# google/lyra

Hardware: NVIDIA H100
Metric: 20ms-frame encode+decode throughput (frames/s) @16kHz (higher is better)
Workload: dtype f32+i8 (decoder fp32 GEMMs: split tf32 on tensor cores)

## Files before the change

include/lyra_b200.h:

```cpp
#ifndef LYRA_B200_H_
#define LYRA_B200_H_

#include <stdint.h>

#ifdef __cplusplus
extern "C" {
#endif

#define LYRA_B200_OK 0
#define LYRA_B200_EINVAL (-1)
#define LYRA_B200_ENODEV (-2)
#define LYRA_B200_EMODEL (-3)

#define LYRA_B200_HOP 320
#define LYRA_B200_NUM_FEATURES 64
#define LYRA_B200_MAX_BITS 184
#define LYRA_B200_MAX_STAGES 46

typedef struct lyra_b200_ctx lyra_b200_ctx;

int lyra_b200_create(const char* model_dir, int device, int max_streams, lyra_b200_ctx** out);
#define LYRA_B200_ROLE_ENCODER 1
#define LYRA_B200_ROLE_DECODER 2
int lyra_b200_create_ex(const char* model_dir, int device, int max_streams, int roles, lyra_b200_ctx** out);
// ... 78 lines not shown
                              int32_t* d_indices );
int lyra_b200_dequantize_device(lyra_b200_ctx* ctx, int n, const uint8_t* d_packets, int num_bits, float* d_features);
int lyra_b200_generate_device(lyra_b200_ctx* ctx, int n, const float* d_features , int16_t* d_pcm );
int lyra_b200_logmel_device(lyra_b200_ctx* ctx, int bank, int n, const int16_t* d_pcm, int num_mel_bins, float* d_out);
int lyra_b200_noise_estimate_device(lyra_b200_ctx* ctx, int n, float* d_noise_estimate ,
                                    uint8_t* d_is_noise );
int lyra_b200_cng_generate_device(lyra_b200_ctx* ctx, int n, const float* d_features , int16_t* d_pcm );
int lyra_b200_resample_device(lyra_b200_ctx* ctx, int to_internal, int n, int external_rate_hz, const int16_t* d_in, int in_samples,
                              int16_t* d_out, int out_stride, int32_t* d_out_counts );
int lyra_b200_set_active_mask(lyra_b200_ctx* ctx, const uint8_t* d_active);
#define LYRA_B200_STATS_WORDS 8
#define LYRA_B200_STAT_HOPS 0
#define LYRA_B200_STAT_SAT_OUT 1
#define LYRA_B200_STAT_ENERGY 2
#define LYRA_B200_STAT_LEVEL 3
#define LYRA_B200_STAT_EMPTY 4
#define LYRA_B200_STAT_BITS 5
#define LYRA_B200_STAT_RECEIVED 4
#define LYRA_B200_STAT_CN_HOPS 5
#define LYRA_B200_STAT_EVENTS 6
int lyra_b200_set_stats(lyra_b200_ctx* ctx, int enable);
int lyra_b200_read_stats(lyra_b200_ctx* ctx, int role, const int32_t* stream_ids, int n, uint64_t* stats , int clear);
int lyra_b200_read_stats_device(lyra_b200_ctx* ctx, int role, int n, uint64_t* d_stats , int clear);
int lyra_b200_synchronize(lyra_b200_ctx* ctx);
int lyra_b200_set_split(lyra_b200_ctx* ctx, int parts);
#define LYRA_B200_DECODER_EXACT 0
#define LYRA_B200_DECODER_TENSOR 1
int lyra_b200_set_decoder_mode(lyra_b200_ctx* ctx, int mode);
int lyra_b200_decoder_mode(const lyra_b200_ctx* ctx);
int lyra_b200_set_blocking_sync(lyra_b200_ctx* ctx, int enable);
int lyra_b200_set_priority(lyra_b200_ctx* ctx, int priority);
int lyra_b200_set_graphs(lyra_b200_ctx* ctx, int enable);
uint64_t lyra_b200_graph_replays(const lyra_b200_ctx* ctx);
uint64_t lyra_b200_launch_count(const lyra_b200_ctx* ctx);

#define LYRA_B200_NUM_KERNELS 8
int lyra_b200_profile_enable(lyra_b200_ctx* ctx, int enable);
int lyra_b200_profile_read(lyra_b200_ctx* ctx, double* ms_sum, uint64_t* launches);

#ifdef __cplusplus
}
#endif
#endif
```

lyra_b200/_capi.py:

```python
import ctypes as C
import os

import numpy as np

_HERE = os.path.dirname(os.path.abspath(__file__))
PRODUCT_SO = os.path.join(_HERE, "liblyra_b200.so")
MODEL_DIR = os.path.join(_HERE, "model_coeffs")

OK, EINVAL, ENODEV, EMODEL = 0, -1, -2, -3
HOP = 320
STATS_WORDS = 8
STAT_HOPS, STAT_SAT_OUT, STAT_ENERGY, STAT_LEVEL = 0, 1, 2, 3
STAT_EMPTY, STAT_BITS = 4, 5
STAT_RECEIVED, STAT_CN_HOPS, STAT_EVENTS = 4, 5, 6
NUM_FEATURES = 64
MAX_STAGES = 46


class LyraB200Error(RuntimeError):
    def __init__(self, code, msg):
        super().__init__("lyra_b200 error %d: %s" % (code, msg))
        self.code = code


class CApi:
    def __init__(self, so_path):
        if not os.path.exists(so_path):
            raise FileNotFoundError(
                "%s not found: the CUDA extension is not built (python -c 'import __graft_entry__ as g; g.build()')" % so_path)
        L = C.CDLL(so_path)
        vp, ci = C.c_void_p, C.c_int
        sig = {
            "lyra_b200_create": (ci, [C.c_char_p, ci, ci, C.POINTER(vp)]),
            "lyra_b200_create_ex": (ci, [C.c_char_p, ci, ci, ci, C.POINTER(vp)]),
            "lyra_b200_destroy": (None, [vp]),
            "lyra_b200_last_error": (C.c_char_p, [vp]),
            "lyra_b200_max_streams": (ci, [vp]),
            "lyra_b200_tile_streams": (ci, [vp]),
            "lyra_b200_reset": (ci, [vp, vp, ci]),
            "lyra_b200_encode": (ci, [vp, vp, ci, vp, ci, vp]),
            "lyra_b200_decode": (ci, [vp, vp, ci, vp, vp, ci, vp]),
            "lyra_b200_extract_features": (ci, [vp, vp, ci, vp, vp]),
            "lyra_b200_quantize": (ci, [vp, ci, vp, ci, vp, vp]),
            "lyra_b200_dequantize": (ci, [vp, ci, vp, ci, vp]),
            "lyra_b200_generate": (ci, [vp, vp, ci, vp, vp]),
            "lyra_b200_logmel": (ci, [vp, ci, vp, ci, vp, ci, vp]),
            "lyra_b200_set_stream": (ci, [vp, vp]),
            "lyra_b200_encode_device": (ci, [vp, ci, vp, ci, vp]),
            "lyra_b200_decode_device": (ci, [vp, ci, vp, vp, ci, vp]),
            "lyra_b200_synchronize": (ci, [vp]),
            "lyra_b200_noise_update": (ci, [vp, vp, ci, vp, vp, vp, vp]),
            "lyra_b200_decode_track_noise": (ci, [vp, vp, ci, vp, vp, ci, vp, vp]),
            "lyra_b200_decode_track_noise_device": (ci, [vp, ci, vp, vp, ci, vp, vp]),
            "lyra_b200_noise_update_device": (ci, [vp, ci, vp, vp, vp, vp]),
            "lyra_b200_set_split": (ci, [vp, ci]),
            "lyra_b200_set_blocking_sync": (ci, [vp, ci]),
            "lyra_b200_set_graphs": (ci, [vp, ci]),
            "lyra_b200_set_priority": (ci, [vp, ci]),
            "lyra_b200_graph_replays": (C.c_uint64, [vp]),
            "lyra_b200_set_decoder_mode": (ci, [vp, ci]),
            "lyra_b200_decoder_mode": (ci, [vp]),
            "lyra_b200_launch_count": (C.c_uint64, [vp]),
            "lyra_b200_profile_enable": (ci, [vp, ci]),
            "lyra_b200_profile_read": (ci, [vp, vp, vp]),
            "lyra_b200_noise_estimate": (ci, [vp, vp, ci, vp, vp]),
            "lyra_b200_decode_plc": (ci, [vp, vp, ci, vp, vp, ci, vp, vp]),
            "lyra_b200_decode_plc_device": (ci, [vp, ci, vp, vp, ci, vp, vp]),
            "lyra_b200_plc_get_state": (ci, [vp, vp, ci, vp]),
            "lyra_b200_plc_set_state": (ci, [vp, vp, ci, vp]),
            "lyra_b200_cng_generate": (ci, [vp, vp, ci, vp, vp]),
            "lyra_b200_set_cng_seed": (ci, [vp, C.c_uint64]),
            "lyra_b200_encode_dtx": (ci, [vp, vp, ci, vp, ci, vp, vp]),
            "lyra_b200_encode_dtx_device": (ci, [vp, ci, vp, ci, vp, vp]),
            "lyra_b200_set_active_mask": (ci, [vp, vp]),
            "lyra_b200_set_stats": (ci, [vp, ci]),
            "lyra_b200_read_stats": (ci, [vp, ci, vp, ci, vp, ci]),
            "lyra_b200_read_stats_device": (ci, [vp, ci, ci, vp, ci]),
            "lyra_b200_resample": (ci, [vp, ci, vp, ci, ci, vp, ci, vp, ci, vp]),
            "lyra_b200_set_sample_rate": (ci, [vp, ci]),
            "lyra_b200_sample_rate": (ci, [vp]),
            "lyra_b200_set_stream_sample_rates": (ci, [vp, vp, ci, vp]),
            "lyra_b200_stream_sample_rates": (ci, [vp, vp, ci, vp]),
            "lyra_b200_set_stream_bits": (ci, [vp, ci, vp, ci, vp]),
            "lyra_b200_stream_bits": (ci, [vp, ci, vp, ci, vp]),
            "lyra_b200_set_stream_dtx": (ci, [vp, vp, ci, vp]),
            "lyra_b200_stream_dtx": (ci, [vp, vp, ci, vp]),
            "lyra_b200_stream_state_bytes": (ci, [vp]),
            "lyra_b200_export_streams": (ci, [vp, vp, ci, vp]),
            "lyra_b200_import_streams": (ci, [vp, vp, ci, vp]),
            "lyra_b200_copy_streams": (ci, [vp, vp, vp, ci]),
            "lyra_b200_align_streams": (ci, [vp, vp, vp, ci]),
            "lyra_b200_extract_features_device": (ci, [vp, ci, vp, vp]),
            "lyra_b200_quantize_device": (ci, [vp, ci, vp, ci, vp, vp]),
            "lyra_b200_dequantize_device": (ci, [vp, ci, vp, ci, vp]),
            "lyra_b200_generate_device": (ci, [vp, ci, vp, vp]),
            "lyra_b200_logmel_device": (ci, [vp, ci, ci, vp, ci, vp]),
            "lyra_b200_noise_estimate_device": (ci, [vp, ci, vp, vp]),
            "lyra_b200_cng_generate_device": (ci, [vp, ci, vp, vp]),
            "lyra_b200_resample_device": (ci, [vp, ci, ci, ci, vp, ci, vp, ci, vp]),
        }
        for name, (res, args) in sig.items():
            fn = getattr(L, name)
            fn.restype = res
            fn.argtypes = args
        self.lib = L
        self.path = so_path

    EXPORTS = ["lyra_b200_create", "lyra_b200_create_ex", "lyra_b200_destroy", "lyra_b200_last_error", "lyra_b200_max_streams",
               "lyra_b200_tile_streams", "lyra_b200_reset", "lyra_b200_encode", "lyra_b200_decode",
               "lyra_b200_extract_features", "lyra_b200_quantize", "lyra_b200_dequantize", "lyra_b200_generate",
               "lyra_b200_logmel", "lyra_b200_set_stream", "lyra_b200_encode_device", "lyra_b200_decode_device",
               "lyra_b200_synchronize", "lyra_b200_noise_update", "lyra_b200_noise_update_device", "lyra_b200_decode_track_noise",
               "lyra_b200_decode_track_noise_device", "lyra_b200_set_split", "lyra_b200_set_blocking_sync", "lyra_b200_set_graphs", "lyra_b200_set_priority", "lyra_b200_graph_replays", "lyra_b200_set_decoder_mode", "lyra_b200_decoder_mode", "lyra_b200_launch_count", "lyra_b200_profile_enable",
               "lyra_b200_profile_read", "lyra_b200_noise_estimate", "lyra_b200_decode_plc", "lyra_b200_decode_plc_device",
               "lyra_b200_plc_get_state", "lyra_b200_plc_set_state", "lyra_b200_cng_generate", "lyra_b200_set_cng_seed",
               "lyra_b200_encode_dtx", "lyra_b200_encode_dtx_device", "lyra_b200_set_active_mask", "lyra_b200_set_stats",
               "lyra_b200_read_stats", "lyra_b200_read_stats_device", "lyra_b200_resample", "lyra_b200_set_sample_rate",
               "lyra_b200_sample_rate", "lyra_b200_set_stream_sample_rates", "lyra_b200_stream_sample_rates", "lyra_b200_set_stream_bits",
               "lyra_b200_stream_bits", "lyra_b200_set_stream_dtx", "lyra_b200_stream_dtx", "lyra_b200_stream_state_bytes", "lyra_b200_export_streams", "lyra_b200_import_streams",
               "lyra_b200_copy_streams", "lyra_b200_align_streams", "lyra_b200_extract_features_device", "lyra_b200_quantize_device",
               "lyra_b200_dequantize_device", "lyra_b200_generate_device", "lyra_b200_logmel_device", "lyra_b200_noise_estimate_device",
               "lyra_b200_cng_generate_device", "lyra_b200_resample_device"]


_product = None


def load():
    global _product
    if _product is None:
        _product = CApi(PRODUCT_SO)
    return _product


def _ptr(a):
    return None if a is None else a.ctypes.data_as(C.c_void_p)


def _ids(stream_ids, n):
    if stream_ids is None:
        return None
    a = np.ascontiguousarray(stream_ids, dtype=np.int32)
    if a.size != n:
        raise ValueError("stream_ids must have one id per row")
    return a

# ... 318 lines not shown
                                                           C.c_void_p(d_indices or 0)))

    def dequantize_device(self, n, d_packets, num_bits, d_features):
        self._check(self.api.lib.lyra_b200_dequantize_device(self.h, n, C.c_void_p(d_packets), num_bits, C.c_void_p(d_features)))

    def generate_device(self, n, d_features, d_pcm):
        self._check(self.api.lib.lyra_b200_generate_device(self.h, n, C.c_void_p(d_features), C.c_void_p(d_pcm)))

    def logmel_device(self, n, d_pcm, d_out, num_mel_bins=160, bank=0):
        self._check(self.api.lib.lyra_b200_logmel_device(self.h, bank, n, C.c_void_p(d_pcm), num_mel_bins, C.c_void_p(d_out)))

    def noise_estimate_device(self, n, d_estimate, d_is_noise):
        self._check(self.api.lib.lyra_b200_noise_estimate_device(self.h, n, C.c_void_p(d_estimate or 0), C.c_void_p(d_is_noise or 0)))

    def cng_generate_device(self, n, d_features, d_pcm):
        self._check(self.api.lib.lyra_b200_cng_generate_device(self.h, n, C.c_void_p(d_features), C.c_void_p(d_pcm)))

    def resample_device(self, n, external_rate_hz, to_internal, d_in, in_samples, d_out, out_stride, d_counts=0):
        self._check(self.api.lib.lyra_b200_resample_device(self.h, 1 if to_internal else 0, n, int(external_rate_hz), C.c_void_p(d_in),
                                                           in_samples, C.c_void_p(d_out), out_stride, C.c_void_p(d_counts or 0)))

    def synchronize(self):
        self._check(self.api.lib.lyra_b200_synchronize(self.h))

    def set_decoder_mode(self, mode):
        self._check(self.api.lib.lyra_b200_set_decoder_mode(self.h, {"exact": 0, "tensor": 1}[mode]))

    def set_blocking_sync(self, enable):
        self._check(self.api.lib.lyra_b200_set_blocking_sync(self.h, 1 if enable else 0))

    def set_graphs(self, enable):
        self._check(self.api.lib.lyra_b200_set_graphs(self.h, 1 if enable else 0))

    def set_priority(self, priority):
        self._check(self.api.lib.lyra_b200_set_priority(self.h, int(priority)))

    def graph_replays(self):
        return int(self.api.lib.lyra_b200_graph_replays(self.h))

    def set_split(self, parts):
        self._check(self.api.lib.lyra_b200_set_split(self.h, int(parts)))

    KERNEL_NAMES = ["EncoderKernelA", "EncoderKernelB", "RvqEncodeKernel", "RvqDecodeKernel", "DecoderKernelC",
                    "DecoderKernelD", "LogMelKernel", "NoiseEstimatorKernel"]

    def profile_enable(self, enable=True):
        self._check(self.api.lib.lyra_b200_profile_enable(self.h, 1 if enable else 0))

    def profile_read(self):
        ms = (C.c_double * len(self.KERNEL_NAMES))()
        cnt = (C.c_uint64 * len(self.KERNEL_NAMES))()
        self._check(self.api.lib.lyra_b200_profile_read(self.h, ms, cnt))
        return {k: (ms[i], int(cnt[i])) for i, k in enumerate(self.KERNEL_NAMES)}
```

lyra_b200/csrc/aux_kernels.cuh:

```cuda
#pragma once

#include "kernel_prims.cuh"
#include "net_kernels.cuh"

namespace lyra_b200 {

constexpr int kRvqBitsPerStage = 4;

struct RowIo {
  const int* ids;
  int slot0, slots;
  const uint8_t* active;
  __device__ __forceinline__ int Stream(int slot) const { return ids ? ids[slot] : slot; }
  __device__ __forceinline__ bool SatOut(int slot) const { return active != nullptr && !active[slot]; }
};

struct StreamWords {
  const int* rate;
  int ctx_rate;
  const int* bits;
  const int* dtx_off;
  __device__ __forceinline__ int Rate(int stream) const {
    if (!rate) return ctx_rate;
    const int w = rate[stream];
    return w ? w : ctx_rate;
  }
  __device__ __forceinline__ int Stages(int stream, int nq) const {
    if (!bits) return nq;
    const int w = bits[stream];
    return w ? w / kRvqBitsPerStage : nq;
  }
  __device__ __forceinline__ bool DtxOff(int stream) const { return dtx_off != nullptr && dtx_off[stream] != 0; }
};

constexpr int kRvqThreads = 128;
constexpr int kRvqSlotsPerBlock = kRvqThreads / 16;

__global__ void __launch_bounds__(kRvqThreads)
RvqEncodeKernel(const uint8_t* __restrict__ blob, RvqParams P, const __grid_constant__ RowIo io, const __grid_constant__ StreamWords words,
                const float* __restrict__ features, int nq, uint8_t* __restrict__ packets, int packet_bytes, int* __restrict__ indices_out,
                const uint8_t* __restrict__ skip) {
  unsigned char* smem = LYRA_DYN_SMEM();
  float* cbs = reinterpret_cast<float*>(smem);
  float* rs = cbs + 2 * 1024;
  int* idxs = reinterpret_cast<int*>(rs + kRvqSlotsPerBlock * 64);
  const int tid = (int)threadIdx.x, grp = tid / 16, c = tid % 16;
  const int row = (int)blockIdx.x * kRvqSlotsPerBlock + grp, slot = io.slot0 + row;
  const bool valid = row < io.slots;
  const int my_nq = valid ? words.Stages(io.Stream(slot), nq) : 0;
  int block_nq = nq;
  if (words.bits) {
    block_nq = 0;
    for (int g = 0; g < kRvqSlotsPerBlock; ++g) {
      const int r = (int)blockIdx.x * kRvqSlotsPerBlock + g;
      if (r < io.slots) block_nq = max(block_nq, words.Stages(io.Stream(io.slot0 + r), nq));
    }
  }
  const bool skipped = valid && (io.SatOut(slot) || (skip != nullptr && skip[slot]));
  float* r = rs + grp * 64;
  int* idx = idxs + grp * 48;
  const float* cbt = BlobPtr<float>(blob, P.codebooks_t);
  LYRA_STATIC_SMEM(LyraMbar, full, 2);
  if (tid == 0) {
    lyra_mbar_init(&full[0], 1);
    lyra_mbar_init(&full[1], 1);
    lyra_mbar_fence_init();
    lyra_bulk_g2s(cbs, cbt, 4096u, &full[0]);
  }
  for (int jj = 0; jj < 4; ++jj) r[c + 16 * jj] = valid ? features[(size_t)slot * 64 + c + 16 * jj] : 0.0f;
  for (int s = 0; s < block_nq; ++s) {
    __syncthreads();
    if (tid == 0 && s + 1 < block_nq) lyra_bulk_g2s(cbs + ((s + 1) & 1) * 1024, cbt + (size_t)(s + 1) * 1024, 4096u, &full[(s + 1) & 1]);
    lyra_mbar_wait(&full[s & 1], (unsigned)((s >> 1) & 1));
    const float* cs = cbs + (s & 1) * 1024 + c;
    float d = 0.0f;
#pragma unroll 16
    for (int j = 0; j < 64; ++j) {
      const float df = __fsub_rn(r[j], cs[j * 16]);
      d = __fadd_rn(d, __fmul_rn(df, df));
    }
    int best = c;
#pragma unroll
    for (int m = 8; m >= 1; m >>= 1) {
      const float od = __shfl_xor_sync(0xffffffffu, d, m, 16);
      const int oi = __shfl_xor_sync(0xffffffffu, best, m, 16);
      if (od < d || (od == d && oi < best)) { d = od; best = oi; }
    }
    __syncwarp();
    const float* q = cbs + (s & 1) * 1024 + best;
#pragma unroll
    for (int jj = 0; jj < 4; ++jj) {
      const int j = c + 16 * jj;
      const float rj = r[j];
      const float t = __fsub_rn(q[j * 16], rj);
      const float u = __fadd_rn(rj, t);
      r[j] = __fsub_rn(rj, u);
    }
    if (c == 0) idx[s] = best;
  }
  __syncthreads();
  if (valid) {
    for (int b = c; b < packet_bytes; b += 16) {
      const int hi = 2 * b < my_nq ? idx[2 * b] : 0, lo = 2 * b + 1 < my_nq ? idx[2 * b + 1] : 0;
      packets[(size_t)slot * packet_bytes + b] = skipped ? (uint8_t)0 : (uint8_t)((hi << 4) | lo);
    }
    if (indices_out)
      for (int s = c; s < P.num_stages; s += 16) indices_out[(size_t)slot * P.num_stages + s] = s < my_nq ? idx[s] : -1;
  }
}

__global__ void __launch_bounds__(256)
RvqDecodeKernel(const uint8_t* __restrict__ blob, RvqParams P, const __grid_constant__ RowIo io, const __grid_constant__ StreamWords words,
                const uint8_t* __restrict__ packets, int packet_bytes, const uint8_t* __restrict__ received, int nq,
                float* __restrict__ features, int16_t* __restrict__ sat_out_pcm) {
  const int gid = (int)(blockIdx.x * blockDim.x + threadIdx.x);
  const int row = gid / 64, j = gid % 64, slot = io.slot0 + row;
  if (row >= io.slots) return;
  nq = words.Stages(io.Stream(slot), nq);
  float out = 0.0f;
  const bool sat_out = io.SatOut(slot);
  if (sat_out && sat_out_pcm)
    for (int k = j; k < 320; k += 64) sat_out_pcm[(size_t)slot * 320 + k] = 0;
  if (!sat_out && (received == nullptr || received[slot])) {
    const float* cb = BlobPtr<float>(blob, P.codebooks);
    const uint8_t* pk = packets + (size_t)slot * packet_bytes;
    for (int k = 0; k < P.num_stages; ++k) {
      float t;
      if (k < nq) {
        const int byte = pk[k >> 1];
        const int idx = (k & 1) ? (byte & 15) : (byte >> 4);
        t = __fmul_rn(cb[((size_t)k * 16 + idx) * 64 + j], 1.0f);
      } else {
        t = __fmul_rn(cb[((size_t)k * 16) * 64 + j], 0.0f);
      }
      out = k == 0 ? t : __fadd_rn(out, t);
    }
  }
  features[(size_t)slot * 64 + j] = out;
}

enum StreamStateKind { kStatePlain = 0, kStateCodecRs0 = 1, kStateCodecRs1 = 2, kStateCng = 3 };
constexpr uint32_t kStateMagic = 0x5453594Cu;
constexpr uint32_t kStateVersion = 3;
constexpr int kStateHeaderWords = 16;
enum { kHdrMagic = 0, kHdrVersion, kHdrBytes, kHdrRoles, kHdrRate, kHdrZero5, kHdrModelLo, kHdrModelHi, kHdrLive0, kHdrLive1,
       kHdrKeyLo, kHdrKeyHi };
constexpr int kStateMaxEntries = 27;
// ... 462 lines not shown
```

lyra_b200/csrc/device_compat.h:

```cpp
#pragma once

#ifdef LYRA_EMU
#include "cuda_emu.h"
#define LYRA_DYN_SMEM() (reinterpret_cast<unsigned char*>(cuda_emu::g_blk->smem))
#define LYRA_LAUNCH(kernel, grid, block, smem, stream, ...) \
  cuda_emu::launch((grid), (block), (smem), [&]() { kernel(__VA_ARGS__); })
#define LYRA_SET_MAX_SMEM(kernel, bytes) (0)
#define LYRA_DEVICE_CODE 1
#define LYRA_TRAP() std::abort()
#define __grid_constant__
#else
#include <cuda_runtime.h>
#define LYRA_DYN_SMEM() (lyra_dyn_smem_raw)
#define LYRA_LAUNCH(kernel, grid, block, smem, stream, ...) kernel<<<(grid), (block), (smem), (stream)>>>(__VA_ARGS__)
#define LYRA_SET_MAX_SMEM(kernel, bytes) \
  cudaFuncSetAttribute((kernel), cudaFuncAttributeMaxDynamicSharedMemorySize, (int)(bytes))
#define LYRA_TRAP() __trap()
#ifdef __CUDACC__
extern __shared__ __align__(1024) unsigned char lyra_dyn_smem_raw[];
#endif
#endif

#include <stdint.h>

#if defined(LYRA_EMU)
static inline void lyra_cp_async16(void* smem_dst, const void* gmem_src) { std::memcpy(smem_dst, gmem_src, 16); }
static inline void lyra_cp_async_commit() {}
template <int N>
static inline void lyra_cp_async_wait() {}
#elif defined(__CUDACC__)
__device__ __forceinline__ void lyra_cp_async16(void* smem_dst, const void* gmem_src) {
  const unsigned s = (unsigned)__cvta_generic_to_shared(smem_dst);
  asm volatile("cp.async.cg.shared.global [%0], [%1], 16;\n" ::"r"(s), "l"(gmem_src) : "memory");
}
__device__ __forceinline__ void lyra_cp_async_commit() { asm volatile("cp.async.commit_group;\n" ::: "memory"); }
template <int N>
__device__ __forceinline__ void lyra_cp_async_wait() { asm volatile("cp.async.wait_group %0;\n" ::"n"(N) : "memory"); }
#endif

struct alignas(8) LyraMbar { unsigned long long v; };
#if defined(LYRA_EMU)
struct LyraMbarEmu { uint16_t expected, arrived, phase, pad; };
static inline LyraMbarEmu* lyra_mbar_emu(LyraMbar* b) { return reinterpret_cast<LyraMbarEmu*>(b); }
static inline void lyra_mbar_init(LyraMbar* b, unsigned count) { LyraMbarEmu* e = lyra_mbar_emu(b); e->expected = (uint16_t)count; e->arrived = 0; e->phase = 0; e->pad = 0; }
static inline void lyra_mbar_fence_init() {}
static inline void lyra_fence_proxy_async() {}
static inline void lyra_mbar_arrive(LyraMbar* b) {
// ... 20 lines not shown
__device__ __forceinline__ unsigned lyra_smem_u32(const void* p) { return (unsigned)__cvta_generic_to_shared(p); }
__device__ __forceinline__ void lyra_mbar_init(LyraMbar* b, unsigned count) {
  asm volatile("mbarrier.init.shared::cta.b64 [%0], %1;\n" ::"r"(lyra_smem_u32(b)), "r"(count) : "memory");
}
__device__ __forceinline__ void lyra_mbar_fence_init() {
  asm volatile("fence.mbarrier_init.release.cluster;\n" ::: "memory");
  asm volatile("fence.proxy.async.shared::cta;\n" ::: "memory");
}
__device__ __forceinline__ void lyra_fence_proxy_async() { asm volatile("fence.proxy.async.shared::cta;\n" ::: "memory"); }
__device__ __forceinline__ void lyra_mbar_arrive(LyraMbar* b) {
  asm volatile("mbarrier.arrive.shared::cta.b64 _, [%0];\n" ::"r"(lyra_smem_u32(b)) : "memory");
}
__device__ __forceinline__ void lyra_mbar_arrive_n(LyraMbar* b, unsigned n) {
  asm volatile("mbarrier.arrive.shared::cta.b64 _, [%0], %1;\n" ::"r"(lyra_smem_u32(b)), "r"(n) : "memory");
}
__device__ __forceinline__ void lyra_bulk_g2s(void* smem_dst, const void* gmem_src, unsigned bytes, LyraMbar* b) {
  const unsigned bar = lyra_smem_u32(b);
  asm volatile("mbarrier.arrive.expect_tx.shared::cta.b64 _, [%0], %1;\n" ::"r"(bar), "r"(bytes) : "memory");
  asm volatile("cp.async.bulk.shared::cluster.global.mbarrier::complete_tx::bytes [%0], [%1], %2, [%3];\n"
               ::"r"(lyra_smem_u32(smem_dst)), "l"(gmem_src), "r"(bytes), "r"(bar) : "memory");
}
__device__ __forceinline__ void lyra_mbar_wait(LyraMbar* b, unsigned parity) {
  const unsigned bar = lyra_smem_u32(b);
  asm volatile("{\n"
               ".reg .pred p;\n"
               "LYRA_WAIT:\n"
               "mbarrier.try_wait.parity.shared::cta.b64 p, [%0], %1;\n"
               "@p bra LYRA_DONE;\n"
               "bra LYRA_WAIT;\n"
               "LYRA_DONE:\n"
               "}\n" ::"r"(bar), "r"(parity) : "memory");
}
#define LYRA_STATIC_SMEM(type, name, count) __shared__ type name##_storage[count]; type* name = name##_storage
#endif

#if defined(LYRA_EMU)
static inline void lyra_mma_s8_16x8x32(int (&c)[4], const uint32_t (&a)[4], const uint32_t (&b)[2]) {
  const uint32_t mine[6] = {a[0], a[1], a[2], a[3], b[0], b[1]};
  const uint32_t (*all)[8] = cuda_emu::warp_gather(mine, 6);
  const int lane = (int)(threadIdx.x & 31), g = lane >> 2, t = lane & 3;
  auto A = [&](int row, int k) {
    const int src = (row & 7) * 4 + (k & 15) / 4;
    const int reg = (row >> 3) + 2 * (k >> 4);
    return (int)(int8_t)((all[src][reg] >> (8 * (k & 3))) & 0xff);
  };
  auto B = [&](int k, int col) {
    const int src = col * 4 + (k & 15) / 4;
    return (int)(int8_t)((all[src][4 + (k >> 4)] >> (8 * (k & 3))) & 0xff);
  };
  int d[4] = {c[0], c[1], c[2], c[3]};
  for (int k = 0; k < 32; ++k) {
    d[0] += A(g, k) * B(k, 2 * t);
    d[1] += A(g, k) * B(k, 2 * t + 1);
    d[2] += A(g + 8, k) * B(k, 2 * t);
    d[3] += A(g + 8, k) * B(k, 2 * t + 1);
  }
  cuda_emu::warp_barrier();
  c[0] = d[0]; c[1] = d[1]; c[2] = d[2]; c[3] = d[3];
}
#elif defined(__CUDACC__)
__device__ __forceinline__ void lyra_mma_s8_16x8x32(int (&c)[4], const uint32_t (&a)[4], const uint32_t (&b)[2]) {
  asm volatile("mma.sync.aligned.m16n8k32.row.col.s32.s8.s8.s32 {%0,%1,%2,%3}, {%4,%5,%6,%7}, {%8,%9}, {%0,%1,%2,%3};\n"
               : "+r"(c[0]), "+r"(c[1]), "+r"(c[2]), "+r"(c[3])
               : "r"(a[0]), "r"(a[1]), "r"(a[2]), "r"(a[3]), "r"(b[0]), "r"(b[1]));
}
#endif
// ... 127 lines not shown
```

lyra_b200/csrc/engine.cu:

```cuda
#include <cmath>
#include <cstdio>
#include <cstdlib>
#include <cstring>
#include <string>
#include <vector>

#include "../../include/lyra_b200.h"
#include "aux_kernels.cuh"
#include "model_spec.h"
#include "net_kernels.cuh"
#include "net_kernels_wgmma.cuh"
#include "plc_kernels.cuh"

using namespace lyra_b200;

namespace {

std::string g_create_error;

#define CU(call)                                                                        \
  do {                                                                                  \
    cudaError_t e_ = (call);                                                            \
    if (e_ != cudaSuccess) {                                                            \
      ctx->err = std::string(#call) + ": " + cudaGetErrorString(e_);                    \
// ... 87 lines not shown
  int* h_slot_of[2] = {nullptr, nullptr};
  cudaEvent_t ev_map[2] = {nullptr, nullptr};
  bool map_pending[2] = {false, false};
  int map_buf = 0;
  std::vector<uint32_t> tile_gen;
  uint32_t map_gen = 0;
  std::vector<uint32_t> id_seen;
  uint32_t id_gen = 0;
  std::vector<int> touched[2];
  int map_dense_n = -1;
  int active_tiles = 0;
  cudaStream_t own_stream = nullptr, stream = nullptr;
  static constexpr int kMaxSplit = 4;
  cudaStream_t aux_stream[kMaxSplit - 1] = {nullptr, nullptr, nullptr};
  cudaEvent_t ev_fork = nullptr, ev_join[kMaxSplit - 1] = {nullptr, nullptr, nullptr};
  int nsplit = 3;
  bool blocking_sync = false;
  cudaEvent_t ev_sync = nullptr;
  int decoder_mode = LYRA_B200_DECODER_EXACT;
  int priority = 0;
  uint64_t launches = 0;
  struct GraphKey {
    int kind, n, num_bits, mode, nsplit;
    const void *a, *b, *c;
    bool rates, bits, stats;
    bool operator==(const GraphKey& o) const {
      return kind == o.kind && n == o.n && num_bits == o.num_bits && mode == o.mode && nsplit == o.nsplit && a == o.a && b == o.b && c == o.c &&
             rates == o.rates && bits == o.bits && stats == o.stats;
    }
  };
  struct GraphEntry { GraphKey key; void* exec; uint64_t launches; };
  bool use_graphs = false;
  std::vector<GraphEntry> graphs;
  uint64_t graph_replays = 0;
  std::string err;
  bool profiling = false;
  std::vector<std::pair<cudaEvent_t, cudaEvent_t>> prof_events[LYRA_B200_NUM_KERNELS];
  size_t prof_used[LYRA_B200_NUM_KERNELS] = {};
  double prof_ms[LYRA_B200_NUM_KERNELS] = {};
  uint64_t prof_n[LYRA_B200_NUM_KERNELS] = {};
};

namespace {

int PacketBytes(int num_bits) { return (num_bits + 7) / 8; }

int RatePair(int rate_hz) { return rate_hz == 8000 ? 0 : rate_hz == 32000 ? 1 : rate_hz == 48000 ? 2 : -1; }
bool RateOk(int rate_hz) { return rate_hz == 16000 || RatePair(rate_hz) >= 0; }

bool Converts(const lyra_b200_ctx* ctx) { return ctx->sample_rate != 16000 || ctx->rate_override; }

NoiseParams MakeNoiseParams(int rate_hz) {
  NoiseParams p{};
  const float secs_per_hop = static_cast<float>(320) / rate_hz;
  p.nf = 160;
  p.hops_per_update = (int)std::round(1.f / secs_per_hop);
  p.max_smoothing = std::pow(0.5f, secs_per_hop / 0.7f);
  p.bound_decay = std::pow(0.5f, secs_per_hop / 1.f);
  p.log_nf = std::log((double)160);
  return p;
}

constexpr int kNoProf = -1;
struct ProfScope {
  lyra_b200_ctx* ctx;
  int k;
  cudaEvent_t stop = nullptr;
  cudaStream_t st;
  ProfScope(lyra_b200_ctx* c, int kernel, cudaStream_t stream) : ctx(c), k(kernel), st(stream) {
    if (!ctx->profiling || k == kNoProf) return;
    auto& pool = ctx->prof_events[k];
    if (ctx->prof_used[k] == pool.size()) {
      cudaEvent_t a, b;
      cudaEventCreate(&a);
      cudaEventCreate(&b);
      pool.emplace_back(a, b);
    }
    auto& ev = pool[ctx->prof_used[k]++];
    cudaEventRecord(ev.first, st);
    stop = ev.second;
  }
  ~ProfScope() { if (stop) cudaEventRecord(stop, st); }
};

template <typename Fn>
int Launch(lyra_b200_ctx* ctx, int prof, cudaStream_t st, Fn launch) {
  {
    ProfScope ps(ctx, prof, st);
    launch();
  }
  ctx->launches += 1;
  CU(cudaGetLastError());
  return LYRA_B200_OK;
}
#define LAUNCH(prof, kernel, grid, block, smem, st, ...) \
  Launch(ctx, (prof), (st), [&]() { LYRA_LAUNCH(kernel, grid, block, smem, st, __VA_ARGS__); })

void ProfDrain(lyra_b200_ctx* ctx) {
  for (int k = 0; k < LYRA_B200_NUM_KERNELS; ++k) {
    for (size_t i = 0; i < ctx->prof_used[k]; ++i) {
      float ms = 0.0f;
      if (cudaEventElapsedTime(&ms, ctx->prof_events[k][i].first, ctx->prof_events[k][i].second) == cudaSuccess) {
        ctx->prof_ms[k] += ms;
        ctx->prof_n[k] += 1;
      }
    }
    ctx->prof_used[k] = 0;
  }
}

cudaError_t SyncStream(lyra_b200_ctx* ctx) {
  if (!ctx->blocking_sync) return cudaStreamSynchronize(ctx->stream);
  cudaError_t e = cudaEventRecord(ctx->ev_sync, ctx->stream);
  return e != cudaSuccess ? e : cudaEventSynchronize(ctx->ev_sync);
}

bool UseDevice(lyra_b200_ctx* ctx) {
  if (cudaSetDevice(ctx->device) == cudaSuccess) return true;
  ctx->err = "cudaSetDevice failed";
  return false;
}

bool RoleOk(lyra_b200_ctx* ctx, int role) {
  if (ctx->roles & role) return true;
  ctx->err = role == LYRA_B200_ROLE_ENCODER ? "this context was created without the encoder role" : "this context was created without the decoder role";
  return false;
}

bool BitsOk(lyra_b200_ctx* ctx, int num_bits) {
// ... 55 lines not shown
  for (int k = 0; k < n; ++k) {
    const int id = ids ? ids[k] : k;
    slot_of[id] = k;
    ctx->touched[b].push_back(id);
  }
  if (++ctx->map_gen == 0) { std::fill(ctx->tile_gen.begin(), ctx->tile_gen.end(), 0u); ctx->map_gen = 1; }
  for (int k = 0; k < n; ++k) {
    const int t = (ids ? ids[k] : k) / kTileStreams;
    if (ctx->tile_gen[(size_t)t] != ctx->map_gen) { ctx->tile_gen[(size_t)t] = ctx->map_gen; tile_list[ntl++] = t; }
  }
  ctx->active_tiles = ntl;
  CU(cudaMemcpyAsync(ctx->d_slot_of, slot_of, sizeof(int) * (size_t)ctx->padded, cudaMemcpyHostToDevice, ctx->stream));
  CU(cudaMemcpyAsync(ctx->d_tile_list, tile_list, sizeof(int) * (size_t)ntl, cudaMemcpyHostToDevice, ctx->stream));
  CU(cudaEventRecord(ctx->ev_map[b], ctx->stream));
  ctx->map_pending[b] = true;
  ctx->map_buf = b ^ 1;
  ctx->map_dense_n = ids ? -1 : n;
  return LYRA_B200_OK;
}

struct Part {
  int tile0, ntiles, slot0, nslots;
  cudaStream_t st;
};
Part WholeCall(lyra_b200_ctx* ctx, int n) { return Part{0, ctx->active_tiles, 0, n, ctx->stream}; }

RowIo Rows(const Part& p, const int* ids, const uint8_t* active) { return RowIo{ids, p.slot0, p.nslots, active}; }

constexpr StreamWords kWords16k{nullptr, 16000, nullptr, nullptr};

int LaunchEncoderNets(lyra_b200_ctx* ctx, const Part& p, const uint8_t* skip, const int16_t* d_pcm, float* d_features,
                      const uint8_t* active) {
  const TileIo io{ctx->d_tile_list + p.tile0, ctx->d_slot_of, skip, active};
  const int rc = LAUNCH(0, EncoderKernelA, dim3((unsigned)p.ntiles), dim3(EncA::NT), (size_t)EncA::kSmemBytes, p.st,
                        ctx->d_blob, ctx->spec.enc, io, d_pcm, reinterpret_cast<float*>(ctx->d_state[0]), ctx->d_n18[0], ctx->d_mid_enc);
  return rc ? rc : LAUNCH(1, EncoderKernelB, dim3((unsigned)p.ntiles), dim3(EncB::NT), (size_t)EncB::kSmemBytes, p.st,
                          ctx->d_blob, ctx->spec.enc, io, ctx->d_mid_enc, reinterpret_cast<float*>(ctx->d_state[1]), ctx->d_n18[1], d_features);
}

int LaunchQuantize(lyra_b200_ctx* ctx, cudaStream_t st, const RowIo& io, const StreamWords& words, const float* d_features, int num_bits,
                   uint8_t* d_packets, int* d_indices, const uint8_t* d_skip) {
  const int nq = num_bits / ctx->spec.bits_per_stage, pb = PacketBytes(num_bits);
  const int blocks = (io.slots + kRvqSlotsPerBlock - 1) / kRvqSlotsPerBlock;
  return LAUNCH(2, RvqEncodeKernel, dim3((unsigned)blocks), dim3(kRvqThreads), (size_t)(2 * 1024 * 4 + kRvqSlotsPerBlock * (64 * 4 + 48 * 4)), st,
                ctx->d_blob, ctx->spec.rvq, io, words, d_features, nq, d_packets, pb, d_indices, d_skip);
}

int LaunchDequantize(lyra_b200_ctx* ctx, cudaStream_t st, const RowIo& io, const StreamWords& words, const uint8_t* d_packets,
                     const uint8_t* d_received, int num_bits, float* d_features, int16_t* sat_out_pcm) {
  const int nq = num_bits / ctx->spec.bits_per_stage, pb = PacketBytes(num_bits);
  const int blocks = (io.slots * 64 + 255) / 256;
  return LAUNCH(3, RvqDecodeKernel, dim3((unsigned)blocks), dim3(256), (size_t)0, st,
                ctx->d_blob, ctx->spec.rvq, io, words, d_packets, pb, d_received, nq, d_features, sat_out_pcm);
}

int LaunchDecoderNets(lyra_b200_ctx* ctx, const Part& p, const uint8_t* skip, const float* d_features, int16_t* d_pcm,
                      const uint8_t* active) {
  const TileIo io{ctx->d_tile_list + p.tile0, ctx->d_slot_of, skip, active};
  const bool tc = ctx->decoder_mode == LYRA_B200_DECODER_TENSOR;
  const dim3 grid((unsigned)p.ntiles);
  float* st_c = reinterpret_cast<float*>(ctx->d_state[2]);
  float* st_d = reinterpret_cast<float*>(ctx->d_state[3]);
  const int rc = tc ? LAUNCH(4, DecoderKernelC<true>, grid, dim3(DecC<true>::NT), (size_t)DecC<true>::kSmemBytes, p.st,
                             ctx->d_blob, ctx->spec.dec, io, d_features, st_c, ctx->d_n18[2], ctx->d_mid_dec)
                    : LAUNCH(4, DecoderKernelC<false>, grid, dim3(DecC<false>::NT), (size_t)DecC<false>::kSmemBytes, p.st,
                             ctx->d_blob, ctx->spec.dec, io, d_features, st_c, ctx->d_n18[2], ctx->d_mid_dec);
  if (rc) return rc;
  return tc ? LAUNCH(5, DecoderKernelDW, grid, dim3(DecDW::NT), (size_t)DecDW::kSmemBytes, p.st,
                     ctx->d_blob, ctx->spec.dec, io, ctx->d_mid_dec, st_d, ctx->d_n18[3], d_pcm)
            : LAUNCH(5, DecoderKernelD, grid, dim3(DecD::NT), (size_t)DecD::kSmemBytes, p.st,
                     ctx->d_blob, ctx->spec.dec, io, ctx->d_mid_dec, st_d, ctx->d_n18[3], d_pcm);
}

int SplitParts(lyra_b200_ctx* ctx, int n, Part* parts) {
  int np = ctx->nsplit < 1 ? 1 : (ctx->nsplit > lyra_b200_ctx::kMaxSplit ? lyra_b200_ctx::kMaxSplit : ctx->nsplit);
  if (!(ctx->map_dense_n == n && ctx->active_tiles >= 64 * np)) np = 1;
  if (np == 1) { parts[0] = WholeCall(ctx, n); return 1; }
  for (int i = 0; i < np; ++i) {
    const int t0 = (int)((long long)ctx->active_tiles * i / np), t1 = (int)((long long)ctx->active_tiles * (i + 1) / np);
    const int s0 = t0 * kTileStreams, s1 = i + 1 == np ? n : t1 * kTileStreams;
    parts[i] = Part{t0, t1 - t0, s0, s1 - s0, i == 0 ? ctx->stream : ctx->aux_stream[i - 1]};
  }
  return np;
}
int Fork(lyra_b200_ctx* ctx, int nparts) {
  if (nparts < 2) return LYRA_B200_OK;
  CU(cudaEventRecord(ctx->ev_fork, ctx->stream));
  for (int i = 1; i < nparts; ++i) CU(cudaStreamWaitEvent(ctx->aux_stream[i - 1], ctx->ev_fork, 0));
  return LYRA_B200_OK;
}
int Join(lyra_b200_ctx* ctx, int nparts) {
  for (int i = 1; i < nparts; ++i) {
    CU(cudaEventRecord(ctx->ev_join[i - 1], ctx->aux_stream[i - 1]));
    CU(cudaStreamWaitEvent(ctx->stream, ctx->ev_join[i - 1], 0));
  }
  return LYRA_B200_OK;
}
int JoinAfter(lyra_b200_ctx* ctx, int nparts, int rc) {
  if (!rc) return Join(ctx, nparts);
  const std::string first = ctx->err;
  Join(ctx, nparts);
  cudaStreamSynchronize(ctx->stream);
  ctx->err = first;
// ... 1000 lines not shown
  return LYRA_B200_OK;
}

int lyra_b200_encode_device(lyra_b200_ctx* ctx, int n, const int16_t* d_pcm, int num_bits, uint8_t* d_packets) {
  if (!ctx || !d_pcm || !d_packets) return LYRA_B200_EINVAL;
  CodecCall c{kEncode, n, num_bits};
  c.dev.pcm_in = d_pcm;
  c.dev.packets_out = d_packets;
  return RunCodecCall(ctx, c);
}

int lyra_b200_decode_device(lyra_b200_ctx* ctx, int n, const uint8_t* d_packets, const uint8_t* d_received, int num_bits,
                            int16_t* d_pcm) {
  if (!ctx || !d_packets || !d_pcm) return LYRA_B200_EINVAL;
  CodecCall c{kDecode, n, num_bits};
  c.dev.packets_in = d_packets;
  c.dev.received = d_received;
  c.dev.pcm_out = d_pcm;
  return RunCodecCall(ctx, c);
}

int lyra_b200_set_graphs(lyra_b200_ctx* ctx, int enable) {
  if (!ctx) return LYRA_B200_EINVAL;
  ENTER(0);
#ifndef LYRA_EMU
  CU(SyncStream(ctx));
  if (!enable) DropGraphs(ctx);
#endif
  ctx->use_graphs = enable != 0;
  return LYRA_B200_OK;
}
uint64_t lyra_b200_graph_replays(const lyra_b200_ctx* ctx) { return ctx ? ctx->graph_replays : 0; }

int lyra_b200_encode(lyra_b200_ctx* ctx, const int32_t* ids, int n, const int16_t* pcm, int num_bits, uint8_t* packets) {
  if (!ctx || !pcm || !packets) return LYRA_B200_EINVAL;
  CodecCall c{kEncode, n, num_bits, ids};
  c.host.pcm_in = pcm;
  c.host.packets_out = packets;
  return RunCodecCall(ctx, c);
}

int lyra_b200_decode(lyra_b200_ctx* ctx, const int32_t* ids, int n, const uint8_t* packets, const uint8_t* received,
                     int num_bits, int16_t* pcm) {
  if (!ctx || !packets || !pcm) return LYRA_B200_EINVAL;
  CodecCall c{kDecode, n, num_bits, ids};
  c.host.packets_in = packets;
  c.host.received = received;
  c.host.pcm_out = pcm;
  return RunCodecCall(ctx, c);
}

int lyra_b200_extract_features(lyra_b200_ctx* ctx, const int32_t* ids, int n, const int16_t* pcm, float* features) {
  if (!ctx || !pcm || !features) return LYRA_B200_EINVAL;
  int rc = CheckNets(ctx, LYRA_B200_ROLE_ENCODER, ids, n);
  if (rc) return rc;
  CU(cudaMemcpyAsync(ctx->d_pcm, pcm, sizeof(int16_t) * 320 * (size_t)n, cudaMemcpyHostToDevice, ctx->stream));
  if ((rc = LaunchEncoderNets(ctx, WholeCall(ctx, n), nullptr, ctx->d_pcm, ctx->d_features, nullptr))) return rc;
  CU(cudaMemcpyAsync(features, ctx->d_features, sizeof(float) * 64 * (size_t)n, cudaMemcpyDeviceToHost, ctx->stream));
  CU(SyncStream(ctx));
  return LYRA_B200_OK;
}

int lyra_b200_extract_features_device(lyra_b200_ctx* ctx, int n, const int16_t* d_pcm, float* d_features) {
  if (!ctx || !d_pcm || !d_features) return LYRA_B200_EINVAL;
  const int rc = CheckNets(ctx, LYRA_B200_ROLE_ENCODER, nullptr, n);
  return rc ? rc : ForEachPart(ctx, n, [&](const Part& p) { return LaunchEncoderNets(ctx, p, nullptr, d_pcm, d_features, nullptr); });
// ... 365 lines not shown
```

lyra_b200/csrc/net_kernels.cuh:

```cuda
#pragma once

#include <type_traits>

#include "kernel_prims.cuh"

namespace lyra_b200 {

constexpr int kTileStreams = 8;

struct EncStateA {
  static constexpr int kFirst = 0;
  static constexpr int kRing0 = 48, kRing1 = kRing0 + 64 * 2, kRing2 = kRing1 + 64 * 6;
  static constexpr int kDown0 = kRing2 + 64 * 18;
  static constexpr int kUnits = kDown0 + 64 * 5;
  static constexpr int kT = 20;
};
struct EncStateB {
  static constexpr int kRing0 = 0, kRing1 = 128 * 2, kRing2 = kRing1 + 128 * 6;
  static constexpr int kDown1 = kRing2 + 128 * 18;
  static constexpr int kRingM = kDown1 + 128 * 2;
  static constexpr int kRingQ0 = kRingM + 256 * 2;
  static constexpr int kRingQ1 = kRingQ0 + 64 * 6;
  static constexpr int kDown2 = kRingQ1 + 64 * 18;
  static constexpr int kBott = kDown2 + 64 * 2;
// ... 54 lines not shown
  const uint8_t* skip;
  const uint8_t* active;
};

template <int S>
__device__ __forceinline__ void LoadTileMeta(const TileIo& io, const int* n18_global, int* slot, int* active, int* n18, int& tile) {
  tile = io.tile_list[blockIdx.x];
  if ((int)threadIdx.x < S) {
    const int stream = tile * S + (int)threadIdx.x;
    const int sl = io.slot_of_stream[stream];
    slot[threadIdx.x] = sl;
    active[threadIdx.x] = sl >= 0 && !(io.active != nullptr && !io.active[sl]) && !(io.skip != nullptr && io.skip[sl]);
    n18[threadIdx.x] = n18_global[stream];
  }
  __syncthreads();
  if (threadIdx.x == 0) {
    int u = -2;
    for (int s = 0; s < S; ++s)
      if (active[s]) u = (u == -2 || u == n18[s]) ? n18[s] : -1;
    n18[S] = u;
  }
  __syncthreads();
}
constexpr int kTileIdle = -2;

constexpr int kMax(int a, int b) { return a > b ? a : b; }

__device__ __forceinline__ void PrefetchTileState(const void* p, int bytes) {
  if (threadIdx.x == 0) lyra_prefetch_l2(p, (unsigned)bytes);
}

template <int S>
__device__ __forceinline__ bool BeginTile(const TileIo& io, const int* n18g, int* meta, float* state, int units, int& tile) {
  LoadTileMeta<S>(io, n18g, meta, meta + S, meta + 2 * S, tile);
  if (meta[3 * S] == kTileIdle) return false;
  PrefetchTileState(state + (size_t)tile * units * S, units * S * 4);
  return true;
}

template <int S>
__device__ __forceinline__ void AdvanceHopCounters(int* n18g, int tile, const int* active, const int* n18) {
  const int tid = (int)threadIdx.x;
  if (tid < S && active[tid]) n18g[tile * S + tid] = (n18[tid] + 1) % 18;
}

template <int S, int NT, int C, int R, typename T>
__device__ __forceinline__ void StoreCarriedRows(T* st, int unit, const T* buf, int ld, int row0, const int* active) {
  for (int i = (int)threadIdx.x; i < C * R * S; i += NT) {
    const int c = i / (R * S), r = i % (R * S);
    if (active[r % S]) st[unit * S + i] = buf[(size_t)c * ld + row0 * S + r];
  }
}

template <int S, int NT, int TM, int TN1, int TN2, int WM, int KC, int C, int T, int DIL, bool TC = false, int LDD = T * S,
          int WTM = 1, int WTN = 1, int STG = kStages>
__device__ __forceinline__ void ResUnitF32(const uint8_t* blob, const ResF32& p, float* u, int ldu, int row0u, float* d,
                                           int groups2, float* ring, const int* n18,
                                           const int* active, float* wbuf, bool last, const WNext& after, int dil_rt = DIL) {
  constexpr int ldd = LDD;
  if (n18[S] >= 0) {
    auto dw = [&](auto dil) {
      DwF32RingFast<S, NT, C, T, decltype(dil)::value>(u, ldu, row0u, d, ldd, BlobPtr<float>(blob, p.dw.w), BlobPtr<float>(blob, p.dw.bias), ring, n18[S], active);
    };
    if constexpr (DIL != 0) dw(std::integral_constant<int, DIL>());
    else if (dil_rt == 1) dw(std::integral_constant<int, 1>());
    else if (dil_rt == 3) dw(std::integral_constant<int, 3>());
// ... 670 lines not shown
```

Measured before the change: 4.210 million.

## Enable programmatic dependent launch across the encoder/decoder kernel chain

Launches the encoder, RVQ and decoder kernels with the programmatic stream serialization attribute via cudaLaunchKernelEx. Each kernel calls griddepcontrol.wait before reading anything its predecessor produced. The RVQ encode kernel now starts its codebook bulk copy before that wait, so the weight load overlaps the tail of the previous kernel. The goal is to hide launch latency and prologue time between back-to-back small kernels; overlap is on by default and can be toggled at runtime, which drops cached graphs.

```diff
diff --git a/include/lyra_b200.h b/include/lyra_b200.h
--- a/include/lyra_b200.h
+++ b/include/lyra_b200.h
@@ -134,6 +134,7 @@
 int lyra_b200_set_priority(lyra_b200_ctx* ctx, int priority);
 int lyra_b200_set_graphs(lyra_b200_ctx* ctx, int enable);
 uint64_t lyra_b200_graph_replays(const lyra_b200_ctx* ctx);
+int lyra_b200_set_launch_overlap(lyra_b200_ctx* ctx, int enable);
 uint64_t lyra_b200_launch_count(const lyra_b200_ctx* ctx);
 
 #define LYRA_B200_NUM_KERNELS 8
diff --git a/lyra_b200/_capi.py b/lyra_b200/_capi.py
--- a/lyra_b200/_capi.py
+++ b/lyra_b200/_capi.py
@@ -56,6 +56,7 @@
             "lyra_b200_set_split": (ci, [vp, ci]),
             "lyra_b200_set_blocking_sync": (ci, [vp, ci]),
             "lyra_b200_set_graphs": (ci, [vp, ci]),
+            "lyra_b200_set_launch_overlap": (ci, [vp, ci]),
             "lyra_b200_set_priority": (ci, [vp, ci]),
             "lyra_b200_graph_replays": (C.c_uint64, [vp]),
             "lyra_b200_set_decoder_mode": (ci, [vp, ci]),
@@ -111,7 +112,7 @@
                "lyra_b200_extract_features", "lyra_b200_quantize", "lyra_b200_dequantize", "lyra_b200_generate",
                "lyra_b200_logmel", "lyra_b200_set_stream", "lyra_b200_encode_device", "lyra_b200_decode_device",
                "lyra_b200_synchronize", "lyra_b200_noise_update", "lyra_b200_noise_update_device", "lyra_b200_decode_track_noise",
-               "lyra_b200_decode_track_noise_device", "lyra_b200_set_split", "lyra_b200_set_blocking_sync", "lyra_b200_set_graphs", "lyra_b200_set_priority", "lyra_b200_graph_replays", "lyra_b200_set_decoder_mode", "lyra_b200_decoder_mode", "lyra_b200_launch_count", "lyra_b200_profile_enable",
+               "lyra_b200_decode_track_noise_device", "lyra_b200_set_split", "lyra_b200_set_blocking_sync", "lyra_b200_set_graphs", "lyra_b200_set_launch_overlap", "lyra_b200_set_priority", "lyra_b200_graph_replays", "lyra_b200_set_decoder_mode", "lyra_b200_decoder_mode", "lyra_b200_launch_count", "lyra_b200_profile_enable",
                "lyra_b200_profile_read", "lyra_b200_noise_estimate", "lyra_b200_decode_plc", "lyra_b200_decode_plc_device",
                "lyra_b200_plc_get_state", "lyra_b200_plc_set_state", "lyra_b200_cng_generate", "lyra_b200_set_cng_seed",
                "lyra_b200_encode_dtx", "lyra_b200_encode_dtx_device", "lyra_b200_set_active_mask", "lyra_b200_set_stats",
@@ -496,6 +497,9 @@
     def set_graphs(self, enable):
         self._check(self.api.lib.lyra_b200_set_graphs(self.h, 1 if enable else 0))
 
+    def set_launch_overlap(self, enable):
+        self._check(self.api.lib.lyra_b200_set_launch_overlap(self.h, 1 if enable else 0))
+
     def set_priority(self, priority):
         self._check(self.api.lib.lyra_b200_set_priority(self.h, int(priority)))
 
diff --git a/lyra_b200/csrc/aux_kernels.cuh b/lyra_b200/csrc/aux_kernels.cuh
--- a/lyra_b200/csrc/aux_kernels.cuh
+++ b/lyra_b200/csrc/aux_kernels.cuh
@@ -45,6 +45,15 @@
   float* rs = cbs + 2 * 1024;
   int* idxs = reinterpret_cast<int*>(rs + kRvqSlotsPerBlock * 64);
   const int tid = (int)threadIdx.x, grp = tid / 16, c = tid % 16;
+  const float* cbt = BlobPtr<float>(blob, P.codebooks_t);
+  LYRA_STATIC_SMEM(LyraMbar, full, 2);
+  if (tid == 0) {
+    lyra_mbar_init(&full[0], 1);
+    lyra_mbar_init(&full[1], 1);
+    lyra_mbar_fence_init();
+    lyra_bulk_g2s(cbs, cbt, 4096u, &full[0]);
+  }
+  lyra_grid_dep_wait();
   const int row = (int)blockIdx.x * kRvqSlotsPerBlock + grp, slot = io.slot0 + row;
   const bool valid = row < io.slots;
   const int my_nq = valid ? words.Stages(io.Stream(slot), nq) : 0;
@@ -59,14 +68,6 @@
   const bool skipped = valid && (io.SatOut(slot) || (skip != nullptr && skip[slot]));
   float* r = rs + grp * 64;
   int* idx = idxs + grp * 48;
-  const float* cbt = BlobPtr<float>(blob, P.codebooks_t);
-  LYRA_STATIC_SMEM(LyraMbar, full, 2);
-  if (tid == 0) {
-    lyra_mbar_init(&full[0], 1);
-    lyra_mbar_init(&full[1], 1);
-    lyra_mbar_fence_init();
-    lyra_bulk_g2s(cbs, cbt, 4096u, &full[0]);
-  }
   for (int jj = 0; jj < 4; ++jj) r[c + 16 * jj] = valid ? features[(size_t)slot * 64 + c + 16 * jj] : 0.0f;
   for (int s = 0; s < block_nq; ++s) {
     __syncthreads();
@@ -113,6 +114,7 @@
 RvqDecodeKernel(const uint8_t* __restrict__ blob, RvqParams P, const __grid_constant__ RowIo io, const __grid_constant__ StreamWords words,
                 const uint8_t* __restrict__ packets, int packet_bytes, const uint8_t* __restrict__ received, int nq,
                 float* __restrict__ features, int16_t* __restrict__ sat_out_pcm) {
+  lyra_grid_dep_wait();
   const int gid = (int)(blockIdx.x * blockDim.x + threadIdx.x);
   const int row = gid / 64, j = gid % 64, slot = io.slot0 + row;
   if (row >= io.slots) return;
diff --git a/lyra_b200/csrc/device_compat.h b/lyra_b200/csrc/device_compat.h
--- a/lyra_b200/csrc/device_compat.h
+++ b/lyra_b200/csrc/device_compat.h
@@ -5,6 +5,7 @@
 #define LYRA_DYN_SMEM() (reinterpret_cast<unsigned char*>(cuda_emu::g_blk->smem))
 #define LYRA_LAUNCH(kernel, grid, block, smem, stream, ...) \
   cuda_emu::launch((grid), (block), (smem), [&]() { kernel(__VA_ARGS__); })
+#define LYRA_LAUNCH_PDL(overlap, kernel, grid, block, smem, stream, ...) LYRA_LAUNCH(kernel, grid, block, smem, stream, __VA_ARGS__)
 #define LYRA_SET_MAX_SMEM(kernel, bytes) (0)
 #define LYRA_DEVICE_CODE 1
 #define LYRA_TRAP() std::abort()
@@ -13,6 +14,20 @@
 #include <cuda_runtime.h>
 #define LYRA_DYN_SMEM() (lyra_dyn_smem_raw)
 #define LYRA_LAUNCH(kernel, grid, block, smem, stream, ...) kernel<<<(grid), (block), (smem), (stream)>>>(__VA_ARGS__)
+#define LYRA_LAUNCH_PDL(overlap, kernel, grid_, block_, smem_, stream_, ...)                           \
+  do {                                                                                                 \
+    cudaLaunchAttribute lyra_attr_[1];                                                                 \
+    lyra_attr_[0].id = cudaLaunchAttributeProgrammaticStreamSerialization;                             \
+    lyra_attr_[0].val.programmaticStreamSerializationAllowed = (overlap) ? 1 : 0;                      \
+    cudaLaunchConfig_t lyra_cfg_ = {};                                                                 \
+    lyra_cfg_.gridDim = (grid_);                                                                       \
+    lyra_cfg_.blockDim = (block_);                                                                     \
+    lyra_cfg_.dynamicSmemBytes = (smem_);                                                              \
+    lyra_cfg_.stream = (stream_);                                                                      \
+    lyra_cfg_.attrs = lyra_attr_;                                                                      \
+    lyra_cfg_.numAttrs = 1;                                                                            \
+    cudaLaunchKernelEx(&lyra_cfg_, kernel, __VA_ARGS__);                                               \
+  } while (0)
 #define LYRA_SET_MAX_SMEM(kernel, bytes) \
   cudaFuncSetAttribute((kernel), cudaFuncAttributeMaxDynamicSharedMemorySize, (int)(bytes))
 #define LYRA_TRAP() __trap()
@@ -99,6 +114,12 @@
                "}\n" ::"r"(bar), "r"(parity) : "memory");
 }
 #define LYRA_STATIC_SMEM(type, name, count) __shared__ type name##_storage[count]; type* name = name##_storage
+#endif
+
+#if defined(LYRA_EMU)
+static inline void lyra_grid_dep_wait() {}
+#elif defined(__CUDACC__)
+__device__ __forceinline__ void lyra_grid_dep_wait() { asm volatile("griddepcontrol.wait;\n" ::: "memory"); }
 #endif
 
 #if defined(LYRA_EMU)
diff --git a/lyra_b200/csrc/engine.cu b/lyra_b200/csrc/engine.cu
--- a/lyra_b200/csrc/engine.cu
+++ b/lyra_b200/csrc/engine.cu
@@ -143,6 +143,7 @@
   struct GraphEntry { GraphKey key; void* exec; uint64_t launches; };
   bool use_graphs = false;
   std::vector<GraphEntry> graphs;
+  bool launch_overlap = true;
   uint64_t graph_replays = 0;
   std::string err;
   bool profiling = false;
@@ -206,6 +207,8 @@
 }
 #define LAUNCH(prof, kernel, grid, block, smem, st, ...) \
   Launch(ctx, (prof), (st), [&]() { LYRA_LAUNCH(kernel, grid, block, smem, st, __VA_ARGS__); })
+#define LAUNCH_CHAIN(prof, kernel, grid, block, smem, st, ...) \
+  Launch(ctx, (prof), (st), [&]() { LYRA_LAUNCH_PDL(ctx->launch_overlap, kernel, grid, block, smem, st, __VA_ARGS__); })
 
 void ProfDrain(lyra_b200_ctx* ctx) {
   for (int k = 0; k < LYRA_B200_NUM_KERNELS; ++k) {
@@ -327,9 +330,9 @@
 int LaunchEncoderNets(lyra_b200_ctx* ctx, const Part& p, const uint8_t* skip, const int16_t* d_pcm, float* d_features,
                       const uint8_t* active) {
   const TileIo io{ctx->d_tile_list + p.tile0, ctx->d_slot_of, skip, active};
-  const int rc = LAUNCH(0, EncoderKernelA, dim3((unsigned)p.ntiles), dim3(EncA::NT), (size_t)EncA::kSmemBytes, p.st,
+  const int rc = LAUNCH_CHAIN(0, EncoderKernelA, dim3((unsigned)p.ntiles), dim3(EncA::NT), (size_t)EncA::kSmemBytes, p.st,
                         ctx->d_blob, ctx->spec.enc, io, d_pcm, reinterpret_cast<float*>(ctx->d_state[0]), ctx->d_n18[0], ctx->d_mid_enc);
-  return rc ? rc : LAUNCH(1, EncoderKernelB, dim3((unsigned)p.ntiles), dim3(EncB::NT), (size_t)EncB::kSmemBytes, p.st,
+  return rc ? rc : LAUNCH_CHAIN(1, EncoderKernelB, dim3((unsigned)p.ntiles), dim3(EncB::NT), (size_t)EncB::kSmemBytes, p.st,
                           ctx->d_blob, ctx->spec.enc, io, ctx->d_mid_enc, reinterpret_cast<float*>(ctx->d_state[1]), ctx->d_n18[1], d_features);
 }
 
@@ -337,7 +340,7 @@
                    uint8_t* d_packets, int* d_indices, const uint8_t* d_skip) {
   const int nq = num_bits / ctx->spec.bits_per_stage, pb = PacketBytes(num_bits);
   const int blocks = (io.slots + kRvqSlotsPerBlock - 1) / kRvqSlotsPerBlock;
-  return LAUNCH(2, RvqEncodeKernel, dim3((unsigned)blocks), dim3(kRvqThreads), (size_t)(2 * 1024 * 4 + kRvqSlotsPerBlock * (64 * 4 + 48 * 4)), st,
+  return LAUNCH_CHAIN(2, RvqEncodeKernel, dim3((unsigned)blocks), dim3(kRvqThreads), (size_t)(2 * 1024 * 4 + kRvqSlotsPerBlock * (64 * 4 + 48 * 4)), st,
                 ctx->d_blob, ctx->spec.rvq, io, words, d_features, nq, d_packets, pb, d_indices, d_skip);
 }
 
@@ -345,7 +348,7 @@
                      const uint8_t* d_received, int num_bits, float* d_features, int16_t* sat_out_pcm) {
   const int nq = num_bits / ctx->spec.bits_per_stage, pb = PacketBytes(num_bits);
   const int blocks = (io.slots * 64 + 255) / 256;
-  return LAUNCH(3, RvqDecodeKernel, dim3((unsigned)blocks), dim3(256), (size_t)0, st,
+  return LAUNCH_CHAIN(3, RvqDecodeKernel, dim3((unsigned)blocks), dim3(256), (size_t)0, st,
                 ctx->d_blob, ctx->spec.rvq, io, words, d_packets, pb, d_received, nq, d_features, sat_out_pcm);
 }
 
@@ -356,14 +359,14 @@
   const dim3 grid((unsigned)p.ntiles);
   float* st_c = reinterpret_cast<float*>(ctx->d_state[2]);
   float* st_d = reinterpret_cast<float*>(ctx->d_state[3]);
-  const int rc = tc ? LAUNCH(4, DecoderKernelC<true>, grid, dim3(DecC<true>::NT), (size_t)DecC<true>::kSmemBytes, p.st,
+  const int rc = tc ? LAUNCH_CHAIN(4, DecoderKernelC<true>, grid, dim3(DecC<true>::NT), (size_t)DecC<true>::kSmemBytes, p.st,
                              ctx->d_blob, ctx->spec.dec, io, d_features, st_c, ctx->d_n18[2], ctx->d_mid_dec)
-                    : LAUNCH(4, DecoderKernelC<false>, grid, dim3(DecC<false>::NT), (size_t)DecC<false>::kSmemBytes, p.st,
+                    : LAUNCH_CHAIN(4, DecoderKernelC<false>, grid, dim3(DecC<false>::NT), (size_t)DecC<false>::kSmemBytes, p.st,
                              ctx->d_blob, ctx->spec.dec, io, d_features, st_c, ctx->d_n18[2], ctx->d_mid_dec);
   if (rc) return rc;
-  return tc ? LAUNCH(5, DecoderKernelDW, grid, dim3(DecDW::NT), (size_t)DecDW::kSmemBytes, p.st,
+  return tc ? LAUNCH_CHAIN(5, DecoderKernelDW, grid, dim3(DecDW::NT), (size_t)DecDW::kSmemBytes, p.st,
                      ctx->d_blob, ctx->spec.dec, io, ctx->d_mid_dec, st_d, ctx->d_n18[3], d_pcm)
-            : LAUNCH(5, DecoderKernelD, grid, dim3(DecD::NT), (size_t)DecD::kSmemBytes, p.st,
+            : LAUNCH_CHAIN(5, DecoderKernelD, grid, dim3(DecD::NT), (size_t)DecD::kSmemBytes, p.st,
                      ctx->d_blob, ctx->spec.dec, io, ctx->d_mid_dec, st_d, ctx->d_n18[3], d_pcm);
 }
 
@@ -1430,6 +1433,17 @@
 }
 uint64_t lyra_b200_graph_replays(const lyra_b200_ctx* ctx) { return ctx ? ctx->graph_replays : 0; }
 
+int lyra_b200_set_launch_overlap(lyra_b200_ctx* ctx, int enable) {
+  if (!ctx) return LYRA_B200_EINVAL;
+  ENTER(0);
+#ifndef LYRA_EMU
+  CU(SyncStream(ctx));
+  DropGraphs(ctx);
+#endif
+  ctx->launch_overlap = enable != 0;
+  return LYRA_B200_OK;
+}
+
 int lyra_b200_encode(lyra_b200_ctx* ctx, const int32_t* ids, int n, const int16_t* pcm, int num_bits, uint8_t* packets) {
   if (!ctx || !pcm || !packets) return LYRA_B200_EINVAL;
   CodecCall c{kEncode, n, num_bits, ids};
diff --git a/lyra_b200/csrc/net_kernels.cuh b/lyra_b200/csrc/net_kernels.cuh
--- a/lyra_b200/csrc/net_kernels.cuh
+++ b/lyra_b200/csrc/net_kernels.cuh
@@ -110,6 +110,7 @@
 
 template <int S>
 __device__ __forceinline__ bool BeginTile(const TileIo& io, const int* n18g, int* meta, float* state, int units, int& tile) {
+  lyra_grid_dep_wait();
   LoadTileMeta<S>(io, n18g, meta, meta + S, meta + 2 * S, tile);
   if (meta[3 * S] == kTileIdle) return false;
   PrefetchTileState(state + (size_t)tile * units * S, units * S * 4);
```

New measurement: 4.208 million, median of 6. Within noise of the previous version (-0.1%).
